# V2AI/EFG

Hardware: AMD Instinct MI355X
Metric: scenes/sec ConQueR 1-frame Waymo train step (higher is better)
Workload: dtype f32; 1 GPU; ConQueR res18 p3, 1-sweep Waymo-shaped scenes, 180000 pts/scene, 0.1 m voxels, 2 scenes/GPU, 900 queries, fwd+bwd+AdamW+OneCycle, graph of `value`: FPN levels / heads the reference evaluates and never reads are skipped (same losses and gradients; the line's `full_graph` object times the full reference graph); global_batch=2, parallelism=dp1

## Files before the change

efg_amd/_lib.py:

```python
import ctypes
import os

import torch

_LIB_PATH = os.path.join(os.path.dirname(os.path.abspath(__file__)), "lib", "libefg_hip.so")
_lib = None

c_void_p, c_int, c_int64, c_size_t, c_float = (ctypes.c_void_p, ctypes.c_int, ctypes.c_int64, ctypes.c_size_t,
                                               ctypes.c_float)

_SIGS = {
    "efg_last_error": (ctypes.c_char_p, []),
    "efg_version": (ctypes.c_char_p, []),
    "efg_capture_stream_create": (ctypes.c_int, [ctypes.POINTER(ctypes.c_void_p)]),
    "efg_capture_stream_destroy": (ctypes.c_int, [ctypes.c_void_p]),
    "efg_dynamic_voxelize_f32": (c_int, [c_void_p, c_int64, c_int, c_void_p, c_void_p, c_void_p, c_void_p]),
    "efg_hard_voxelize_workspace_bytes": (c_size_t, [c_int64, c_int, c_int, c_int, c_int, c_void_p, c_void_p]),
    "efg_hard_voxelize_f32": (c_int, [c_void_p, c_void_p, c_int, c_int, c_void_p, c_void_p, c_int, c_int, c_void_p,
                                      c_void_p, c_int, c_void_p, c_void_p, c_void_p, c_void_p, c_size_t, c_void_p]),
    "efg_hard_voxelize_debug_timeline": (c_size_t, [c_void_p]),
    "efg_scatter_workspace_bytes": (c_size_t, [c_int64, c_int, c_void_p]),
    "efg_scatter_index": (c_int, [c_void_p, c_int64, c_int, c_void_p, c_void_p, c_void_p, c_void_p, c_size_t,
                                  c_void_p]),
    "efg_scatter_reduce_workspace_bytes": (c_size_t, [c_int64, c_int]),
    "efg_scatter_reduce_f32": (c_int, [c_void_p, c_void_p, c_void_p, c_int64, c_int, c_int, c_int, c_int64, c_void_p,
                                       c_void_p, c_void_p, c_void_p, c_size_t, c_void_p]),
    "efg_scatter_backward_f32": (c_int, [c_void_p, c_void_p, c_void_p, c_void_p, c_void_p, c_void_p, c_int64, c_int64,
                                         c_int, c_int, c_void_p, c_size_t, c_void_p]),
    "efg_spconv_index_bytes": (c_size_t, [c_int, c_void_p]),
    "efg_spconv_index_workspace_bytes": (c_size_t, [c_int, c_void_p]),
    "efg_spconv_index_from_indices": (c_int, [c_void_p, c_int64, c_int, c_void_p, c_void_p, c_void_p, c_void_p,
                                              c_size_t, c_void_p]),
    "efg_spconv_index_downsample": (c_int, [c_void_p, c_int64, c_int, c_void_p, c_void_p, c_void_p, c_void_p,
                                            c_void_p, c_void_p, c_void_p, c_void_p, c_size_t, c_void_p]),
    "efg_spconv_index_rank": (c_int, [c_void_p, c_int, c_void_p, c_void_p, c_void_p, c_size_t, c_void_p]),
    "efg_spconv_index_emit": (c_int, [c_void_p, c_int, c_void_p, c_void_p, c_void_p]),
    "efg_spconv_build_nbr": (c_int, [c_void_p, c_void_p, c_int, c_void_p, c_void_p, c_int64, c_void_p, c_void_p,
                                     c_void_p, c_void_p, c_void_p]),
    "efg_spconv_build_rnbr": (c_int, [c_void_p, c_int64, c_int, c_int64, c_void_p, c_void_p]),
    "efg_spconv_packed_weight_bytes": (c_size_t, [c_int, c_int, c_int, c_int]),
    "efg_spconv_pack_weight_f32": (c_int, [c_void_p, c_int, c_int, c_int, c_int, c_void_p, c_void_p]),
    "efg_spconv_pack_weights_multi": (c_int, [c_void_p, c_int, c_void_p]),
    "efg_spconv_forward_f32": (c_int, [c_void_p, c_int64, c_int, c_void_p, c_void_p, c_int, c_int, c_void_p, c_int64,
                                       c_void_p, c_void_p]),
    "efg_spconv_dgrad_f32": (c_int, [c_void_p, c_int64, c_int, c_void_p, c_int, c_int, c_void_p, c_int64, c_void_p,
                                     c_void_p, c_void_p]),
    "efg_spconv_tile_plan_bytes": (c_size_t, [c_int64, c_int]),
    "efg_spconv_tile_plan": (c_int, [c_void_p, c_int64, c_int, c_void_p, c_size_t, c_void_p]),
    "efg_spconv_forward_tiled_f32": (c_int, [c_void_p, c_int64, c_int, c_void_p, c_void_p, c_int, c_int, c_void_p,
                                             c_int64, c_int, c_void_p, c_void_p]),
    "efg_spconv_tiled_pair_f32": (c_int, [c_void_p, c_void_p, c_int64, c_int, c_void_p, c_void_p, c_int, c_int, c_void_p,
                                          c_int64, c_int, c_void_p, c_void_p, c_void_p]),
    "efg_spconv_small_ok": (c_int, [c_int, c_int, c_int, c_void_p, c_void_p]),
    "efg_spconv_tile_bf16x3_ok": (c_int, [c_int, c_int, c_int, c_int64, c_int64]),
    "efg_spconv_streamk_fallbacks": (c_int, [c_void_p, c_int]),
    "efg_ticket_ring_errors": (c_int, [c_void_p, c_int]),
    "efg_spconv_parity_order": (c_int, [c_void_p, c_int64, c_void_p, c_void_p, c_size_t, c_void_p]),
    "efg_spconv_wgrad_workspace_bytes": (c_size_t, [c_int64, c_int, c_int, c_int]),
    "efg_spconv_wgrad_f32": (c_int, [c_void_p, c_int64, c_int, c_void_p, c_int64, c_int, c_int, c_void_p, c_void_p,
                                     c_void_p, c_size_t, c_void_p]),
    "efg_spconv_wgrad_tiled_ok": (c_int, [c_int, c_int, c_int]),
    "efg_spconv_wgrad_tiled_workspace_bytes": (c_size_t, [c_int64, c_int, c_int, c_int]),
    "efg_spconv_wgrad_sched_bytes": (c_size_t, [c_int64, c_int, c_int, c_int]),
    "efg_spconv_wgrad_sched": (c_int, [c_void_p, c_int64, c_int, c_int, c_int, c_void_p, c_size_t, c_void_p]),
    "efg_spconv_wgrad_tiled_f32": (c_int, [c_void_p, c_int64, c_int, c_void_p, c_int64, c_int, c_int, c_void_p,
                                           c_void_p, c_void_p, c_void_p, c_size_t, c_void_p]),
    "efg_spconv_wgrad_tiled_pair_f32": (c_int, [c_void_p, c_int64, c_int, c_void_p, c_void_p, c_int64, c_int, c_int, c_void_p,
                                                c_void_p, c_void_p, c_void_p, c_void_p, c_size_t, c_void_p]),
    "efg_sparse_to_dense_f32": (c_int, [c_void_p, c_int, c_void_p, c_void_p, c_int, c_void_p, c_void_p, c_void_p]),
    "efg_dense_to_sparse_f32": (c_int, [c_void_p, c_int, c_void_p, c_int64, c_int, c_void_p, c_void_p, c_void_p]),
    "efg_sparse_to_bev_f32": (c_int, [c_void_p, c_int, c_void_p, c_void_p, c_int, c_void_p, c_void_p, c_void_p]),
    "efg_bev_to_sparse_f32": (c_int, [c_void_p, c_int, c_void_p, c_int64, c_int, c_void_p, c_void_p, c_void_p]),
    "efg_msda_forward_f32": (c_int, [c_void_p, c_void_p, c_void_p, c_void_p, c_void_p, c_int, c_int, c_int, c_int,
                                     c_int, c_int, c_int, c_void_p, c_void_p]),
    "efg_msda_backward_f32": (c_int, [c_void_p, c_void_p, c_void_p, c_void_p, c_void_p, c_void_p, c_int, c_int, c_int,
                                      c_int, c_int, c_int, c_int, c_void_p, c_void_p, c_void_p, c_void_p]),
    "efg_box_attn_fused_forward_f32": (c_int, [c_void_p] * 7 + [c_int] * 8 + [c_void_p, c_void_p]),
    "efg_box_attn_fused_forward_strided_f32": (c_int, [c_void_p] * 5 + [c_int, c_void_p, c_int, c_void_p] + [c_int] * 8 + [c_void_p, c_void_p]),
    "efg_box_attn_fused_backward_strided_f32": (c_int, [c_void_p] * 5 + [c_int, c_void_p, c_int, c_void_p, c_void_p] + [c_int] * 8 + [c_void_p] * 4 + [c_size_t, c_void_p]),
    "efg_box_attn_fused_backward_workspace_bytes": (c_size_t, [c_int] * 6),
    "efg_box_attn_fused_backward_f32": (c_int, [c_void_p] * 8 + [c_int] * 8 + [c_void_p] * 4 + [c_size_t, c_void_p]),
    "efg_boxes_bev_f32": (c_int, [c_void_p, c_int, c_void_p, c_int, c_int, c_void_p, c_void_p]),
    "efg_nms_workspace_bytes": (c_size_t, [c_int]),
    "efg_topk_unsorted_f32": (c_int, [c_void_p, c_int64, c_int, c_int, c_void_p, c_void_p, c_void_p]),
    "efg_box_refine_forward_f32": (c_int, [c_void_p, c_void_p, c_int64, c_float, c_void_p, c_void_p]),
    "efg_box_refine_backward_f32": (c_int, [c_void_p, c_void_p, c_void_p, c_int64, c_float, c_void_p, c_void_p, c_void_p]),
    "efg_add_layernorm_forward_f32": (c_int, [c_void_p] * 4 + [c_float, c_int64, c_int] + [c_void_p] * 5),
    "efg_add_layernorm_backward_workspace_bytes": (c_size_t, [c_int64, c_int]),
    "efg_add_layernorm_backward_f32": (c_int, [c_void_p] * 5 + [c_int64, c_int] + [c_void_p] * 4 + [c_size_t, c_void_p]),
    "efg_points_transform_filter_workspace_bytes": (c_size_t, [c_int64]),
    "efg_points_transform_filter_f32": (c_int, [c_void_p, c_int64, c_int, c_void_p, c_int, c_void_p, c_void_p, c_void_p,
                                                c_void_p, c_size_t, c_void_p]),
    "efg_points_gather_f32": (c_int, [c_void_p, c_void_p, c_int64, c_int, c_void_p, c_void_p]),
    "efg_match_cost_f32": (c_int, [c_void_p] * 4 + [c_int] * 5 + [c_float] * 6 + [c_void_p, c_void_p]),
    "efg_focal_loss_forward_f32": (c_int, [c_void_p, c_void_p, c_int, c_int64, c_int, c_float, c_float, c_void_p, c_void_p,
                                           c_void_p]),
    "efg_focal_loss_backward_f32": (c_int, [c_void_p, c_void_p, c_int, c_int64, c_int, c_float, c_float, c_void_p,
                                            c_void_p, c_void_p, c_void_p]),
    "efg_box_loss_forward_f32": (c_int, [c_void_p] * 6 + [c_int64] + [c_int] * 4 + [c_void_p] * 3),
    "efg_box_loss_backward_f32": (c_int, [c_void_p] * 6 + [c_int64] + [c_int] * 4 + [c_void_p] * 4),
    "efg_bn_workspace_bytes": (c_size_t, [c_int]),
    "efg_bn_forward_f32": (c_int, [c_void_p] * 7 + [c_float, c_float, c_int64, c_int, c_int] + [c_void_p] * 4 +
                           [c_size_t, c_void_p]),
    "efg_bn_backward_f32": (c_int, [c_void_p] * 6 + [c_int64, c_int, c_int] + [c_void_p] * 5 + [c_size_t, c_void_p]),
    "efg_lsap_f32": (c_int, [c_void_p, c_int, c_int, c_int, c_void_p, c_void_p, c_void_p, c_void_p]),
    "efg_nms_f32": (c_int, [c_void_p, c_int, c_float, c_int, c_void_p, c_void_p, c_void_p, c_size_t, c_void_p]),
    "efg_spconv_tile_shape": (c_int, [c_int, c_int, c_int, c_int64, c_int64, c_void_p, c_void_p, c_void_p]),
    "efg_cylinder_select_f32": (c_int, [c_void_p, c_int64, c_int, c_int, c_float, c_void_p, c_void_p, c_int64, c_void_p,
                                        c_void_p, c_void_p, c_int, c_void_p, c_void_p]),
    "efg_attention_fwd_f32": (c_int, [c_void_p, c_int64, c_int64, c_void_p, c_void_p, c_int64, c_int64, c_int64, c_int, c_int,
                                      c_int, c_float, c_void_p, c_void_p, c_void_p]),
    "efg_attention_bwd_f32": (c_int, [c_void_p, c_int64, c_int64, c_void_p, c_void_p, c_int64, c_int64, c_void_p, c_void_p,
                                      c_void_p, c_int64, c_int, c_int, c_int, c_float, c_void_p, c_void_p, c_void_p,
                                      c_void_p]),
    "efg_attention_long_fwd_f32": (c_int, [c_void_p, c_int64, c_int64] * 3 + [c_void_p, c_int, c_int64, c_int, c_int, c_float,
                                                                             c_void_p, c_void_p, c_void_p]),
    "efg_attention_long_bwd_f32": (c_int, [c_void_p, c_int64, c_int64] * 3 + [c_void_p, c_int, c_void_p, c_void_p, c_void_p,
                                                                             c_int64, c_int, c_int, c_float, c_void_p, c_void_p,
                                                                             c_void_p, c_void_p, c_void_p]),
    "efg_relu_bwd_colsum_f32": (c_int, [c_void_p, c_void_p, c_int64, c_int, c_void_p, c_void_p, c_void_p, c_size_t, c_void_p]),
    "efg_nms_segmented_f32": (c_int, [c_void_p, c_void_p, c_int, c_float, c_int, c_void_p, c_void_p, c_void_p, c_size_t,
                                      c_void_p]),
    "efg_gn_workspace_bytes": (c_size_t, [c_int, c_int]),
    "efg_gn_forward_f32": (c_int, [c_void_p] * 3 + [c_float, c_int, c_int64, c_int, c_int] + [c_void_p] * 4 +
                           [c_size_t, c_void_p]),
    "efg_gn_backward_f32": (c_int, [c_void_p] * 5 + [c_int, c_int64, c_int, c_int] + [c_void_p] * 4 +
                            [c_size_t, c_void_p]),
    "efg_gemm_bf16x3_pack_bytes": (c_size_t, [c_int, c_int]),
    "efg_gemm_bf16x3_pack_f32": (c_int, [c_void_p, c_int64, c_int64, c_int, c_int, c_void_p, c_void_p]),
    "efg_gemm_bf16x3_pack_linear_f32": (c_int, [c_void_p, c_int, c_int, c_void_p, c_void_p, c_void_p]),
    "efg_gemm_bf16x3_f32": (c_int, [c_void_p, c_int64, c_int, c_int64, c_void_p, c_int, c_void_p, c_int, c_void_p, c_int64,
                                    c_void_p]),
    "efg_gemm_bf16x3_wgrad_workspace_bytes": (c_size_t, [c_int64, c_int, c_int]),
    "efg_gemm_bf16x3_wgrad_f32": (c_int, [c_void_p, c_int64, c_void_p, c_int64, c_int64, c_int, c_int, c_void_p, c_void_p,
                                          c_size_t, c_void_p]),
    "efg_gemm_bf16x6_pack_bytes": (c_size_t, [c_int, c_int]),
    "efg_gemm_bf16x6_pack_f32": (c_int, [c_void_p, c_int64, c_int64, c_int, c_int, c_void_p, c_void_p]),
    "efg_gemm_bf16x6_pack_linear_f32": (c_int, [c_void_p, c_int, c_int, c_void_p, c_void_p, c_void_p]),
    "efg_gemm_bf16x6_f32": (c_int, [c_void_p, c_int64, c_int, c_int64, c_void_p, c_int, c_void_p, c_int, c_void_p, c_int64,
                                    c_void_p]),
    "efg_gemm_bf16x6_wgrad_workspace_bytes": (c_size_t, [c_int64, c_int, c_int]),
    "efg_gemm_bf16x6_wgrad_f32": (c_int, [c_void_p, c_int64, c_void_p, c_int64, c_int64, c_int, c_int, c_void_p, c_void_p,
                                          c_size_t, c_void_p]),
    "efg_colsum_workspace_bytes": (c_size_t, [c_int64, c_int]),
    "efg_colsum_f32": (c_int, [c_void_p, c_int64, c_int, c_int64, c_void_p, c_void_p, c_size_t, c_void_p]),
}

EXPORTED_SYMBOLS = tuple(_SIGS)


def lib_path():
    return _LIB_PATH


def _warn_if_stale():
    csrc = os.path.join(os.path.dirname(os.path.abspath(__file__)), "csrc")
    try:
        built = os.path.getmtime(_LIB_PATH)
        newer = [f for f in os.listdir(csrc) if os.path.getmtime(os.path.join(csrc, f)) > built + 1.0]
    except OSError:
        return
    if newer:
        import warnings

        warnings.warn("efg_amd: %s is OLDER than %s -- rebuild with `python -m efg_amd.build`"
                      % (os.path.basename(_LIB_PATH), ", ".join(sorted(newer)[:4])), RuntimeWarning, stacklevel=3)


def lib():
    global _lib
    if _lib is None:
        if not os.path.exists(_LIB_PATH):
            raise RuntimeError(
                "efg_amd: %s is missing. Build it with `python -m efg_amd.build` (hipcc, gfx950). "
                "There is no CPU fallback on the product path." % _LIB_PATH)
        _warn_if_stale()
        ab = os.environ.get("EFG_HIP_LIB_AB")
        path = os.path.join(os.path.dirname(_LIB_PATH), os.path.basename(ab)) if ab else _LIB_PATH
        if ab and not os.path.exists(path):
            raise RuntimeError("efg_amd: EFG_HIP_LIB_AB=%s not found in %s" % (ab, os.path.dirname(_LIB_PATH)))
        _lib = ctypes.CDLL(path)
        for name, (res, args) in _SIGS.items():
            fn = getattr(_lib, name)
            fn.restype = res
            fn.argtypes = args
    return _lib


def check(rc):
    if rc != 0:
        raise RuntimeError("efg_hip: " + lib().efg_last_error().decode())


def ptr(t):
    if t is None:
        return None
    assert t.is_contiguous(), "efg_hip ops need contiguous tensors"
    return t.data_ptr()


def stream():
    raw = getattr(torch._C, "_cuda_getCurrentRawStream", None)
    if raw is not None:
        return raw(torch.cuda.current_device())
    return torch.cuda.current_stream().cuda_stream


def require_gpu(*tensors):
    for t in tensors:
        if t is not None and not t.is_cuda:
            raise RuntimeError(
                "efg_amd ops run on MI355X only (got a %s tensor); there is no CPU fallback" % t.device.type)


def host_f32(vals, n):
    vals = [float(v) for v in vals]
    assert len(vals) == n
    return (ctypes.c_float * n)(*vals)


def host_i32(vals, n=None):
    vals = [int(v) for v in vals]
    assert n is None or len(vals) == n
    return (ctypes.c_int * len(vals))(*vals)


def host_i64(vals):
    vals = [int(v) for v in vals]
    return (ctypes.c_int64 * len(vals))(*vals)
```

efg_amd/build.py:

```python
import os
import subprocess
import sys

_PKG = os.path.dirname(os.path.abspath(__file__))
_ROOT = os.path.dirname(_PKG)
CSRC = os.path.join(_PKG, "csrc")
LIB_DIR = os.path.join(_PKG, "lib")
LIB_PATH = os.path.join(LIB_DIR, "libefg_hip.so")

SOURCES = ["lib.cpp", "voxelize.hip", "voxelize_bins.hip", "voxelize_hash.hip", "scatter.hip", "spconv_index.hip", "spconv_conv.hip", "spconv_tiles.hip", "spconv_wgt.hip", "msda.hip", "box_fused.hip", "iou3d_nms.hip", "matcher.hip", "layernorm.hip", "augment.hip", "det_loss.hip", "batchnorm.hip", "colsum.hip", "crop.hip", "attention.hip", "gemm_bf16x3.hip", "gemm_bf16x6.hip", "topk.hip"]
FLAGS = ["--offload-arch=gfx950", "-O3", "-std=c++17", "-fPIC", "-munsafe-fp-atomics", "-ffp-contract=off",
         "-Wall", "-Wno-unused-function", "-I" + os.path.join(_ROOT, "include"), "-I" + CSRC]


def _stale(target, deps):
    if not os.path.exists(target):
        return True
    t = os.path.getmtime(target)
    return any(os.path.getmtime(d) > t for d in deps)


def build(force=False, verbose=False):
    os.makedirs(LIB_DIR, exist_ok=True)
    hipcc = os.environ.get("HIPCC", "/opt/rocm/bin/hipcc")
    headers = [os.path.join(CSRC, h) for h in os.listdir(CSRC) if h.endswith(".h")]
    headers.append(os.path.join(_ROOT, "include", "efg_hip.h"))
    objs = []
    procs = []
    for src in SOURCES:
        path = os.path.join(CSRC, src)
        if not os.path.exists(path):
            continue
        obj = os.path.join(LIB_DIR, os.path.splitext(src)[0] + ".o")
        objs.append(obj)
        if force or _stale(obj, [path] + headers):
            cmd = [hipcc] + FLAGS + ["-x", "hip", "-c", path, "-o", obj]
            if verbose:
                print(" ".join(cmd))
            procs.append((src, subprocess.Popen(cmd, stdout=subprocess.PIPE, stderr=subprocess.STDOUT)))
    for src, p in procs:
        out, _ = p.communicate()
        if p.returncode != 0:
            raise RuntimeError("hipcc failed on %s:\n%s" % (src, out.decode()))
        if verbose and out:
            print(out.decode())
    if force or procs or _stale(LIB_PATH, objs):
        cmd = [hipcc, "--offload-arch=gfx950", "-shared", "-fPIC", "-o", LIB_PATH] + objs
        subprocess.check_call(cmd)
    return LIB_PATH


if __name__ == "__main__":
    print(build(force="--force" in sys.argv, verbose=True))
```

efg_amd/detection3d/optimizer.py:

```python
import torch


class CachedFusedAdamW(torch.optim.AdamW):

    def __init__(self, params, **kw):
        kw["fused"] = True
        super().__init__(params, **kw)
        self._plan = None

    def _plain(self, group):
        return not (group["amsgrad"] or group["maximize"] or group["capturable"] or group["differentiable"]
                    or torch.is_tensor(group["lr"]))

    def _build_plan(self):
        plan = []
        for group in self.param_groups:
            params, grads, exp_avgs, exp_avg_sqs, max_sqs, steps = [], [], [], [], [], []
            self._init_group(group, params, grads, exp_avgs, exp_avg_sqs, max_sqs, steps)
            assert len({(p.device, p.dtype) for p in params}) <= 1, "one device / dtype per group"
            plan.append((params, exp_avgs, exp_avg_sqs, steps))
        return plan

    @torch.no_grad()
    def step(self, closure=None):
        if closure is not None or not all(self._plain(g) for g in self.param_groups):
            return super().step(closure)
        if self._plan is None:
            self._plan = self._build_plan()
        todo = []
        for group, (params, exp_avgs, exp_avg_sqs, steps) in zip(self.param_groups, self._plan):
            grads = [p.grad for p in params]
            if any(g is None for g in grads) or len(params) != sum(p.grad is not None for p in group["params"]):
                self._plan = None
                return super().step()
            todo.append((group, params, grads, exp_avgs, exp_avg_sqs, steps))
        found_inf = getattr(self, "found_inf", None)
        for group, params, grads, exp_avgs, exp_avg_sqs, steps in todo:
            if not params:
                continue
            beta1, beta2 = group["betas"]
            torch._foreach_add_(steps, 1)
            torch._fused_adamw_(params, grads, exp_avgs, exp_avg_sqs, [], steps, amsgrad=False, lr=group["lr"],
                                beta1=beta1, beta2=beta2, weight_decay=group["weight_decay"], eps=group["eps"],
                                maximize=False, grad_scale=None, found_inf=found_inf)
            if found_inf is not None:
                torch._foreach_sub_(steps, [found_inf.reshape(()).to(steps[0].dtype)] * len(steps))
        return None


def build_adamw_multi(cfg, model):
    oc = dict(cfg.solver.optimizer)
    oc.pop("type", None)
    lr = oc["lr"]
    lr_backbone = oc.pop("lr_backbone", lr)
    named = [(n, p) for n, p in model.named_parameters() if p.requires_grad]
    backbone = [p for p in model.backbone.parameters() if p.requires_grad]
    rest = [p for n, p in named if "backbone" not in n and "linear_box" not in n]
    deform = [p for n, p in named if "linear_box" in n and "backbone" not in n]
    groups = [{"params": backbone, "lr": lr_backbone}, {"params": rest},
              {"params": deform, "lr": lr * cfg.solver.deform_lr_multi}]
    oc["betas"] = tuple(oc["betas"])
    if all(p.is_cuda for g in groups for p in g["params"]):
        return CachedFusedAdamW(groups, **oc)
    return torch.optim.AdamW(groups, **oc)
```

include/efg_hip.h:

```cpp
#ifndef EFG_HIP_H
#define EFG_HIP_H
#include <stddef.h>
#include <stdint.h>

#ifdef __cplusplus
extern "C" {
#endif

#define EFG_OK 0
#define EFG_E_INVALID (-1)
#define EFG_E_WORKSPACE (-2)
#define EFG_E_HIP (-3)

const char* efg_last_error(void);
const char* efg_version(void);

int efg_capture_stream_create(void** stream_out);
int efg_capture_stream_destroy(void* stream);


int efg_dynamic_voxelize_f32(const float* points, int64_t n, int f, const float* voxel_size_host,
                             const float* coors_range_host, int32_t* coors, void* stream);

size_t efg_hard_voxelize_workspace_bytes(int64_t n_total, int batch, int f, int max_points, int max_voxels,
                                         const float* voxel_size_host, const float* coors_range_host);

int efg_hard_voxelize_f32(const float* points, const int64_t* point_offsets_host, int batch, int f,
                          const float* voxel_size_host, const float* coors_range_host, int max_points,
                          int max_voxels, float* voxels, int32_t* coors, int coors_cols, int32_t* npv,
                          int32_t* voxel_num, float* mean, void* ws, size_t ws_bytes, void* stream);

size_t efg_hard_voxelize_debug_timeline(void* device_buf_u64);

size_t efg_scatter_workspace_bytes(int64_t n, int ndim, const int32_t* dims_host);
int efg_scatter_index(const int32_t* coors, int64_t n, int ndim, const int32_t* dims_host,
                      int32_t* point2voxel, int32_t* m_dev, void* ws, size_t ws_bytes, void* stream);
size_t efg_scatter_reduce_workspace_bytes(int64_t m, int c);
int efg_scatter_reduce_f32(const float* feats, const int32_t* coors, const int32_t* point2voxel, int64_t n,
                           int c, int ndim, int reduce, int64_t m, float* voxel_feats, int32_t* voxel_coors,
                           int32_t* count, void* ws, size_t ws_bytes, void* stream);
int efg_scatter_backward_f32(float* grad_feats, const float* grad_voxel_feats, const float* feats,
                             const float* voxel_feats, const int32_t* point2voxel, const int32_t* count,
                             int64_t n, int64_t m, int c, int reduce, void* ws, size_t ws_bytes, void* stream);

size_t efg_spconv_index_bytes(int batch, const int* shape_host);
size_t efg_spconv_index_workspace_bytes(int batch, const int* shape_host);

int efg_spconv_index_from_indices(const int32_t* indices, int64_t m, int batch, const int* shape_host,
                                  void* index, int32_t* perm, void* ws, size_t ws_bytes, void* stream);

int efg_spconv_index_downsample(const int32_t* in_indices, int64_t m_in, int batch, const int* in_shape_host,
                                const int* ksize_host, const int* stride_host, const int* pad_host,
                                void* out_index, int* out_shape_host, int32_t* m_out_dev, void* ws,
                                size_t ws_bytes, void* stream);
int efg_spconv_index_rank(void* index, int batch, const int* shape_host, int32_t* m_dev, void* ws, size_t ws_bytes,
                          void* stream);
int efg_spconv_index_emit(const void* index, int batch, const int* shape_host, int32_t* out_indices,
                          void* stream);

int efg_spconv_build_nbr(const void* in_index, const int32_t* in_perm, int batch, const int* in_shape_host,
                         const int32_t* out_indices, int64_t m_out, const int* ksize_host,
                         const int* stride_host, const int* pad_host, int32_t* nbr, void* stream);
int efg_spconv_build_rnbr(const int32_t* nbr, int64_t m_out, int kvol, int64_t m_in, int32_t* rnbr,
                          void* stream);

size_t efg_spconv_packed_weight_bytes(int cout, int kvol, int cin, int for_dgrad);
int efg_spconv_pack_weight_f32(const float* weight, int cout, int kvol, int cin, int for_dgrad, float* packed,
                               void* stream);
int efg_spconv_pack_weights_multi(const void* items_dev, int n, void* stream);

int efg_spconv_forward_f32(const float* in_feat, int64_t m_in, int cin, const float* packed_weight,
                           const float* bias, int cout, int kvol, const int32_t* nbr, int64_t m_out,
                           float* out_feat, void* stream);
int efg_spconv_dgrad_f32(const float* grad_out, int64_t m_out, int cout, const float* packed_weight, int cin,
                         int kvol, const int32_t* rnbr, int64_t m_in, const int32_t* row_order, float* grad_in,
                         void* stream);
size_t efg_spconv_tile_plan_bytes(int64_t m, int kvol);
int efg_spconv_tile_plan(const int32_t* nbr, int64_t m, int kvol, void* plan, size_t plan_bytes, void* stream);
int efg_spconv_tile_shape(int cin, int cout, int kvol, int64_t m_in, int64_t m_out, int* nt, int* r, int* ks);
int efg_spconv_forward_tiled_f32(const float* in_feat, int64_t m_in, int cin, const float* packed_weight,
                                 const float* bias, int cout, int kvol, const void* plan, int64_t m_out,
                                 int flip_offsets, float* out_feat, void* stream);
int efg_spconv_tiled_pair_f32(const float* in_a, const float* in_b, int64_t m_in, int cin, const float* packed_a,
                              const float* packed_b, int cout, int kvol, const void* plan, int64_t m_out, int flip_offsets,
                              float* out_a, float* out_b, void* stream);
int efg_spconv_streamk_fallbacks(int64_t* count_out, int reset);
int efg_spconv_small_ok(int cin, int cout, int kvol, int* c16, int* nt);
int efg_spconv_tile_bf16x3_ok(int cin, int cout, int kvol, int64_t m_in, int64_t m_out);

int efg_spconv_parity_order(const int32_t* indices, int64_t m, int32_t* order, void* ws, size_t ws_bytes,
                            void* stream);
size_t efg_spconv_wgrad_workspace_bytes(int64_t m_out, int cin, int cout, int kvol);
int efg_spconv_wgrad_f32(const float* in_feat, int64_t m_in, int cin, const float* grad_out, int64_t m_out,
                         int cout, int kvol, const int32_t* nbr, float* grad_w, void* ws, size_t ws_bytes,
                         void* stream);
int efg_spconv_wgrad_tiled_ok(int cin, int cout, int kvol);
size_t efg_spconv_wgrad_sched_bytes(int64_t m_out, int cin, int cout, int kvol);
int efg_spconv_wgrad_sched(const void* plan, int64_t m_out, int cin, int cout, int kvol, void* sched, size_t sched_bytes,
                           void* stream);
size_t efg_spconv_wgrad_tiled_workspace_bytes(int64_t m_out, int cin, int cout, int kvol);
int efg_spconv_wgrad_tiled_f32(const float* in_feat, int64_t m_in, int cin, const float* grad_out, int64_t m_out,
                               int cout, int kvol, const void* plan, const void* sched, float* grad_w, void* ws,
                               size_t ws_bytes, void* stream);
int efg_spconv_wgrad_tiled_pair_f32(const float* in_feat, int64_t m_in, int cin, const float* grad_out_a,
                                    const float* grad_out_b, int64_t m_out, int cout, int kvol, const void* plan,
                                    const void* sched, float* grad_w_a, float* grad_w_b, void* ws, size_t ws_bytes,
                                    void* stream);

int efg_sparse_to_dense_f32(const float* feat, int c, const void* index, const int32_t* perm, int batch,
                            const int* shape_host, float* dense, void* stream);
int efg_dense_to_sparse_f32(const float* grad_dense, int c, const int32_t* indices, int64_t m, int batch,
                            const int* shape_host, float* grad_feat, void* stream);

int efg_sparse_to_bev_f32(const float* feat, int c, const void* index, const int32_t* perm, int batch,
                          const int* shape_host, float* out, void* stream);
int efg_bev_to_sparse_f32(const float* grad_out, int c, const int32_t* indices, int64_t m, int batch,
                          const int* shape_host, float* grad_feat, void* stream);

int efg_msda_forward_f32(const float* value, const int64_t* shapes, const int64_t* level_start,
                         const float* loc, const float* attn, int b, int s, int h, int d, int l, int lq, int p,
                         float* out, void* stream);
int efg_msda_backward_f32(const float* value, const int64_t* shapes, const int64_t* level_start,
                          const float* loc, const float* attn, const float* grad_out, int b, int s, int h,
                          int d, int l, int lq, int p, float* grad_value, float* grad_loc, float* grad_attn,
                          void* stream);

int efg_box_attn_fused_forward_f32(const float* value, const int64_t* shapes, const int64_t* level_start,
                                   const float* ref_windows, const float* offsets, const float* logits,
                                   const float* kernel_indices, int b, int s, int h, int d, int l, int lq, int p,
                                   int v, float* out, void* stream);
size_t efg_box_attn_fused_backward_workspace_bytes(int b, int s, int h, int l, int lq, int p);
int efg_box_attn_fused_backward_f32(const float* value, const int64_t* shapes, const int64_t* level_start,
                                    const float* ref_windows, const float* offsets, const float* logits,
                                    const float* kernel_indices, const float* grad_out, int b, int s, int h, int d,
                                    int l, int lq, int p, int v, float* grad_value, float* grad_offsets,
                                    float* grad_logits, void* ws, size_t ws_bytes, void* stream);

int efg_ticket_ring_errors(int64_t* count_out, int reset);

int efg_box_attn_fused_forward_strided_f32(const float* value, const int64_t* shapes, const int64_t* level_start,
                                           const float* ref_windows, const float* offsets, int off_row_stride,
                                           const float* logits, int logit_row_stride, const float* kernel_indices, int b,
                                           int s, int h, int d, int l, int lq, int p, int v, float* out, void* stream);
int efg_box_attn_fused_backward_strided_f32(const float* value, const int64_t* shapes, const int64_t* level_start,
                                            const float* ref_windows, const float* offsets, int off_row_stride,
                                            const float* logits, int logit_row_stride, const float* kernel_indices,
                                            const float* grad_out, int b, int s, int h, int d, int l, int lq, int p, int v,
                                            float* grad_value, float* grad_offsets, float* grad_logits, void* ws,
                                            size_t ws_bytes, void* stream);

int efg_boxes_bev_f32(const float* boxes_a, int na, const float* boxes_b, int nb, int mode, float* out,
                      void* stream);
size_t efg_nms_workspace_bytes(int n);
int efg_nms_f32(const float* boxes_sorted, int n, float thresh, int rotated, int64_t* keep, int* num_keep,
                void* ws, size_t ws_bytes, void* stream);
int efg_nms_segmented_f32(const float* boxes_sorted, const int32_t* segment, int n, float thresh, int rotated,
                          int64_t* keep, int* num_keep, void* ws, size_t ws_bytes, void* stream);

int efg_cylinder_select_f32(const float* points, int64_t n_points, int f, int time_col, float max_time,
                            const int64_t* point_range, const float* centre_radius, int64_t n_cyl, const int64_t* starts,
                            int32_t* counts, int32_t* index, int n_chunks, int32_t* chunk_counts, void* stream);

int efg_attention_fwd_f32(const float* q, int64_t q_batch_stride, int64_t q_row_stride, const float* k, const float* v,
                          int64_t kv_batch_stride, int64_t kv_row_stride, int64_t batch, int seq_q, int seq_k, int heads,
                          float scale, float* out, float* lse, void* stream);
int efg_attention_bwd_f32(const float* q, int64_t q_batch_stride, int64_t q_row_stride, const float* k, const float* v,
                          int64_t kv_batch_stride, int64_t kv_row_stride, const float* out, const float* lse,
                          const float* dout, int64_t batch, int seq_q, int seq_k, int heads, float scale, float* dq, float* dk,
                          float* dv, void* stream);

int efg_attention_long_fwd_f32(const float* q, int64_t q_batch_stride, int64_t q_row_stride, const float* k,
                               int64_t k_batch_stride, int64_t k_row_stride, const float* v, int64_t v_batch_stride,
                               int64_t v_row_stride, const uint32_t* mask_bits, int mask_words, int64_t batch, int s, int heads,
                               float scale, float* out, float* lse, void* stream);
int efg_attention_long_bwd_f32(const float* q, int64_t q_batch_stride, int64_t q_row_stride, const float* k,
                               int64_t k_batch_stride, int64_t k_row_stride, const float* v, int64_t v_batch_stride,
                               int64_t v_row_stride, const uint32_t* mask_bits, int mask_words, const float* out,
                               const float* lse, const float* dout, int64_t batch, int s, int heads, float scale, float* dq,
                               float* dk, float* dv, float* delta_ws , void* stream);

int efg_lsap_f32(const float* cost, int n_problems, int nq, int g_stride, const int32_t* ng,
                 int64_t* query_of_gt, int32_t* status, void* stream);

int efg_add_layernorm_forward_f32(const float* x, const float* residual, const float* gamma, const float* beta,
                                  float eps, int64_t rows, int c, float* z_out, float* y, float* mean, float* rstd,
                                  void* stream);
size_t efg_add_layernorm_backward_workspace_bytes(int64_t rows, int c);
int efg_add_layernorm_backward_f32(const float* dy, const float* z, const float* mean, const float* rstd,
                                   const float* gamma, int64_t rows, int c, float* dz, float* dgamma, float* dbeta,
                                   void* ws, size_t ws_bytes, void* stream);

enum { EFG_PT_NEG_Y = 0,
       EFG_PT_NEG_X = 1,
       EFG_PT_ROT_Z = 2,
       EFG_PT_SCALE = 3,
       EFG_PT_TRANSLATE = 4  };
typedef struct { int kind; float a, b, c; } efg_point_op;
size_t efg_points_transform_filter_workspace_bytes(int64_t n);
int efg_points_transform_filter_f32(const float* points, int64_t n, int f, const efg_point_op* ops_host, int n_ops,
                                    const float* range_host, float* out, int32_t* count, void* ws, size_t ws_bytes,
                                    void* stream);
int efg_points_gather_f32(const float* points, const int64_t* index, int64_t m, int f, float* out, void* stream);

int efg_match_cost_f32(const float* logits, const float* boxes, const int64_t* tgt_labels, const float* tgt_boxes,
                       int p, int b, int q, int c, int g, float w_class, float w_bbox, float w_giou, float w_rad,
                       float alpha, float gamma, float* cost, void* stream);
int efg_focal_loss_forward_f32(const float* logits, const int32_t* target_class, int layers, int64_t n, int c,
                               float alpha, float gamma, const float* denom, float* out, void* stream);
int efg_focal_loss_backward_f32(const float* logits, const int32_t* target_class, int layers, int64_t n, int c,
                                float alpha, float gamma, const float* denom, const float* grad_out,
                                float* grad_logits, void* stream);
int efg_box_loss_forward_f32(const float* boxes, const float* tgt_boxes, const int64_t* l_idx, const int64_t* b_idx,
                             const int64_t* q_idx, const int64_t* g_idx, int64_t n, int layers, int b, int q, int g,
                             const float* denom, float* out, void* stream);
int efg_box_loss_backward_f32(const float* boxes, const float* tgt_boxes, const int64_t* l_idx, const int64_t* b_idx,
                              const int64_t* q_idx, const int64_t* g_idx, int64_t n, int layers, int b, int q, int g,
                              const float* denom, const float* grad_out, float* grad_boxes, void* stream);

int efg_topk_unsorted_f32(const float* x, int64_t rows, int n, int k, float* values, int64_t* indices, void* stream);

int efg_box_refine_forward_f32(const float* delta, const float* anchor, int64_t n, float eps, float* out, void* stream);
int efg_box_refine_backward_f32(const float* grad, const float* out, const float* anchor, int64_t n, float eps,
                                float* grad_delta, float* grad_anchor, void* stream);

size_t efg_bn_workspace_bytes(int c);
int efg_bn_forward_f32(const float* x, const float* residual, const float* weight, const float* bias,
                       float* running_mean, float* running_var, int64_t* num_batches_tracked, float momentum, float eps,
                       int64_t m, int c, int relu, float* y, float* mean, float* invstd, void* ws, size_t ws_bytes,
                       void* stream);
int efg_bn_backward_f32(const float* dy, const float* x, const float* y, const float* weight, const float* mean,
                        const float* invstd, int64_t m, int c, int relu, float* dx, float* dresidual, float* dweight,
                        float* dbias, void* ws, size_t ws_bytes, void* stream);

size_t efg_gn_workspace_bytes(int batch, int c);
int efg_gn_forward_f32(const float* x, const float* weight, const float* bias, float eps, int batch, int64_t rows,
                       int c, int groups, float* y, float* mean, float* rstd, void* ws, size_t ws_bytes, void* stream);
int efg_gn_backward_f32(const float* dy, const float* x, const float* weight, const float* mean, const float* rstd,
                        int batch, int64_t rows, int c, int groups, float* dx, float* dweight, float* dbias, void* ws,
                        size_t ws_bytes, void* stream);

size_t efg_colsum_workspace_bytes(int64_t rows, int cols);
int efg_colsum_f32(const float* x, int64_t rows, int cols, int64_t row_stride, float* out, void* ws, size_t ws_bytes,
                   void* stream);
int efg_relu_bwd_colsum_f32(const float* g, const float* y, int64_t rows, int cols, float* g_out, float* out, void* ws,
                            size_t ws_bytes, void* stream);

size_t efg_gemm_bf16x3_pack_bytes(int k, int n);
int efg_gemm_bf16x3_pack_f32(const float* w, int64_t stride_k, int64_t stride_n, int k, int n, void* packed,
                             void* stream);
int efg_gemm_bf16x3_pack_linear_f32(const float* w, int n_out, int n_in, void* packed_fwd, void* packed_dgrad, void* stream);
int efg_gemm_bf16x3_f32(const float* a, int64_t m, int k, int64_t lda, const void* packed_b, int n, const float* bias,
                        int relu, float* c, int64_t ldc, void* stream);
size_t efg_gemm_bf16x3_wgrad_workspace_bytes(int64_t m, int n, int k);
int efg_gemm_bf16x3_wgrad_f32(const float* g, int64_t ldg, const float* x, int64_t ldx, int64_t m, int n, int k, float* dw,
                              void* ws, size_t ws_bytes, void* stream);

size_t efg_gemm_bf16x6_pack_bytes(int k, int n);
int efg_gemm_bf16x6_pack_f32(const float* w, int64_t stride_k, int64_t stride_n, int k, int n, void* packed,
                             void* stream);
int efg_gemm_bf16x6_pack_linear_f32(const float* w, int n_out, int n_in, void* packed_fwd, void* packed_dgrad, void* stream);
int efg_gemm_bf16x6_f32(const float* a, int64_t m, int k, int64_t lda, const void* packed_b, int n, const float* bias,
                        int relu, float* c, int64_t ldc, void* stream);
size_t efg_gemm_bf16x6_wgrad_workspace_bytes(int64_t m, int n, int k);
int efg_gemm_bf16x6_wgrad_f32(const float* g, int64_t ldg, const float* x, int64_t ldx, int64_t m, int n, int k, float* dw,
                              void* ws, size_t ws_bytes, void* stream);

#ifdef __cplusplus
}
#endif
#endif
```

Before: 64.49 scenes/s.

## Replace per-group fused AdamW with a single custom HIP launch over all params

Adds a HIP AdamW kernel driven by a pinned host table of pointers, per-group scalars and a chunk-to-tensor map, so all parameters are updated in one kernel launch. It replaces the per-group torch foreach step-increment and fused AdamW launches. Step counters are updated in-kernel using atomic tickets so only the last chunk of each tensor writes the step. The cost is a small host-to-device table copy each step, a ring of events to avoid overwriting pinned buffers still in flight, and double-precision coefficient math meant to match PyTorch numerics.

```diff
diff --git a/efg_amd/_lib.py b/efg_amd/_lib.py
--- a/efg_amd/_lib.py
+++ b/efg_amd/_lib.py
@@ -144,6 +144,9 @@
                                           c_size_t, c_void_p]),
     "efg_colsum_workspace_bytes": (c_size_t, [c_int64, c_int]),
     "efg_colsum_f32": (c_int, [c_void_p, c_int64, c_int, c_int64, c_void_p, c_void_p, c_size_t, c_void_p]),
+    "efg_adamw_chunk_elems": (c_int, []),
+    "efg_adamw_table_bytes": (c_size_t, [c_int, c_int, c_int64]),
+    "efg_adamw_step_f32": (c_int, [c_void_p, c_void_p, c_size_t, c_int, c_int, c_int64, c_void_p, c_void_p]),
 }
 
 EXPORTED_SYMBOLS = tuple(_SIGS)
diff --git a/efg_amd/build.py b/efg_amd/build.py
--- a/efg_amd/build.py
+++ b/efg_amd/build.py
@@ -8,7 +8,7 @@
 LIB_DIR = os.path.join(_PKG, "lib")
 LIB_PATH = os.path.join(LIB_DIR, "libefg_hip.so")
 
-SOURCES = ["lib.cpp", "voxelize.hip", "voxelize_bins.hip", "voxelize_hash.hip", "scatter.hip", "spconv_index.hip", "spconv_conv.hip", "spconv_tiles.hip", "spconv_wgt.hip", "msda.hip", "box_fused.hip", "iou3d_nms.hip", "matcher.hip", "layernorm.hip", "augment.hip", "det_loss.hip", "batchnorm.hip", "colsum.hip", "crop.hip", "attention.hip", "gemm_bf16x3.hip", "gemm_bf16x6.hip", "topk.hip"]
+SOURCES = ["lib.cpp", "voxelize.hip", "voxelize_bins.hip", "voxelize_hash.hip", "scatter.hip", "spconv_index.hip", "spconv_conv.hip", "spconv_tiles.hip", "spconv_wgt.hip", "msda.hip", "box_fused.hip", "iou3d_nms.hip", "matcher.hip", "layernorm.hip", "augment.hip", "det_loss.hip", "batchnorm.hip", "colsum.hip", "crop.hip", "attention.hip", "gemm_bf16x3.hip", "gemm_bf16x6.hip", "topk.hip", "adamw.hip"]
 FLAGS = ["--offload-arch=gfx950", "-O3", "-std=c++17", "-fPIC", "-munsafe-fp-atomics", "-ffp-contract=off",
          "-Wall", "-Wno-unused-function", "-I" + os.path.join(_ROOT, "include"), "-I" + CSRC]
 
diff --git a/efg_amd/csrc/adamw.hip b/efg_amd/csrc/adamw.hip
--- /dev/null
+++ b/efg_amd/csrc/adamw.hip
@@ -0,0 +1,125 @@
+#include "common.h"
+
+namespace efg {
+namespace {
+
+constexpr int kChunk = 16384;
+constexpr int kTensorWords = 8;
+constexpr int kGroupWords = 8;
+
+struct Coef {
+  double beta1, beta2, omb1, omb2, lrwd, eps;
+  float step_size, bc2_sqrt;
+  bool decay;
+};
+
+__device__ __forceinline__ void adamw_one(const Coef& k, float& p, float g, float& m, float& v) {
+  const double pd = (double)p, gd = (double)g;
+  if (k.decay) p = (float)__fma_rn(-k.lrwd, pd, pd);
+  m = (float)__fma_rn(k.beta1, (double)m, __dmul_rn(k.omb1, gd));
+  v = (float)__fma_rn(k.beta2, (double)v, __dmul_rn(__dmul_rn(k.omb2, gd), gd));
+  const float denom = (float)__dadd_rn((double)__fdiv_rn(sqrtf(v), k.bc2_sqrt), k.eps);
+  p = __fsub_rn(p, __fdiv_rn(__fmul_rn(k.step_size, m), denom));
+}
+
+__global__ void __launch_bounds__(256)
+adamw_kernel(const long long* __restrict__ table, int T, int G, const float* __restrict__ found_inf,
+             unsigned* __restrict__ tickets) {
+  const float fi = found_inf ? *found_inf : 0.f;
+  if (fi == 1.f) return;
+  const long long* rows = table + (long long)kGroupWords * G;
+  const long long where = rows[(long long)kTensorWords * T + blockIdx.x];
+  const int t = (int)(where & 0xffffffffll), chunk = (int)(where >> 32);
+  const long long numel = rows[5ll * T + t];
+  float* __restrict__ param = reinterpret_cast<float*>(rows[t]);
+  const float* __restrict__ grad = reinterpret_cast<const float*>(rows[1ll * T + t]);
+  float* __restrict__ exp_avg = reinterpret_cast<float*>(rows[2ll * T + t]);
+  float* __restrict__ exp_sq = reinterpret_cast<float*>(rows[3ll * T + t]);
+  float* step_ptr = reinterpret_cast<float*>(rows[4ll * T + t]);
+  const double* grp = reinterpret_cast<const double*>(table) + (long long)kGroupWords * rows[6ll * T + t];
+  const int chunks = (int)rows[7ll * T + t];
+
+  const float step = __fadd_rn(*step_ptr, 1.0f);
+  const double lr = grp[0], wd = grp[3];
+  Coef k;
+  k.beta1 = grp[1];
+  k.beta2 = grp[2];
+  k.omb1 = __dsub_rn(1.0, k.beta1);
+  k.omb2 = __dsub_rn(1.0, k.beta2);
+  k.lrwd = __dmul_rn(lr, wd);
+  k.eps = grp[4];
+  k.decay = wd != 0.0;
+  const float bc1 = (float)__dsub_rn(1.0, pow(k.beta1, (double)step));
+  k.bc2_sqrt = (float)__dsqrt_rn(__dsub_rn(1.0, pow(k.beta2, (double)step)));
+  k.step_size = (float)__ddiv_rn(lr, (double)bc1);
+
+  const long long base = (long long)chunk * kChunk;
+  const int n = (int)min((long long)kChunk, numel - base);
+  param += base;
+  grad += base;
+  exp_avg += base;
+  exp_sq += base;
+  const int n4 = n >> 2;
+  const bool grad_vec = (reinterpret_cast<uintptr_t>(grad) & 15) == 0;
+  for (int i = threadIdx.x; i < n4; i += 256) {
+    float4 p = reinterpret_cast<const float4*>(param)[i];
+    const float4 g = grad_vec ? reinterpret_cast<const float4*>(grad)[i]
+                              : make_float4(grad[4 * i], grad[4 * i + 1], grad[4 * i + 2], grad[4 * i + 3]);
+    float4 m = reinterpret_cast<const float4*>(exp_avg)[i];
+    float4 v = reinterpret_cast<const float4*>(exp_sq)[i];
+    adamw_one(k, p.x, g.x, m.x, v.x);
+    adamw_one(k, p.y, g.y, m.y, v.y);
+    adamw_one(k, p.z, g.z, m.z, v.z);
+    adamw_one(k, p.w, g.w, m.w, v.w);
+    reinterpret_cast<float4*>(param)[i] = p;
+    reinterpret_cast<float4*>(exp_avg)[i] = m;
+    reinterpret_cast<float4*>(exp_sq)[i] = v;
+  }
+  for (int i = (n4 << 2) + threadIdx.x; i < n; i += 256) {
+    float p = param[i], m = exp_avg[i], v = exp_sq[i];
+    adamw_one(k, p, grad[i], m, v);
+    param[i] = p;
+    exp_avg[i] = m;
+    exp_sq[i] = v;
+  }
+
+  __syncthreads();
+  if (threadIdx.x == 0) {
+    bool last = true;
+    if (chunks > 1) {
+      const unsigned prev = __hip_atomic_fetch_add(tickets + t, 1u, __ATOMIC_ACQ_REL, __HIP_MEMORY_SCOPE_AGENT);
+      last = prev == (unsigned)chunks - 1;
+      if (last) __hip_atomic_store(tickets + t, 0u, __ATOMIC_RELAXED, __HIP_MEMORY_SCOPE_AGENT);
+    }
+    if (last) *step_ptr = found_inf ? __fsub_rn(step, fi) : step;
+  }
+}
+
+}
+}
+
+using namespace efg;
+
+extern "C" int efg_adamw_chunk_elems(void) { return kChunk; }
+
+extern "C" size_t efg_adamw_table_bytes(int n_tensors, int n_groups, int64_t n_blocks) {
+  if (n_tensors < 1 || n_groups < 1 || n_blocks < 1) return 0;
+  return sizeof(long long) * ((size_t)kGroupWords * n_groups + (size_t)kTensorWords * n_tensors + (size_t)n_blocks);
+}
+
+extern "C" int efg_adamw_step_f32(const void* host_table, void* dev_table, size_t table_bytes, int n_tensors, int n_groups,
+                                  int64_t n_blocks, const float* found_inf, void* stream) {
+  EFG_CHECK_ARG(n_tensors >= 1 && n_groups >= 1 && n_blocks >= 1 && n_blocks <= 0x7fffffffll,
+                "adamw: need at least one tensor, group and block (got %d, %d, %lld)", n_tensors, n_groups, (long long)n_blocks);
+  EFG_CHECK_ARG(host_table && dev_table, "adamw: null table");
+  EFG_CHECK_ARG(table_bytes == efg_adamw_table_bytes(n_tensors, n_groups, n_blocks), "adamw: table is %zu bytes, expected %zu",
+                table_bytes, efg_adamw_table_bytes(n_tensors, n_groups, n_blocks));
+  hipStream_t st = (hipStream_t)stream;
+  unsigned* tickets = ticket_slots(n_tensors, st);
+  EFG_CHECK_ARG(tickets, "adamw: no ticket slots (more than 2048 tensors, or a stream that is being captured)");
+  EFG_HIP_TRY(hipMemcpyAsync(dev_table, host_table, table_bytes, hipMemcpyHostToDevice, st));
+  hipLaunchKernelGGL(adamw_kernel, dim3((unsigned)n_blocks), dim3(256), 0, st, static_cast<const long long*>(dev_table),
+                     n_tensors, n_groups, found_inf, tickets);
+  EFG_LAUNCH_CHECK();
+  return EFG_OK;
+}
diff --git a/efg_amd/detection3d/optimizer.py b/efg_amd/detection3d/optimizer.py
--- a/efg_amd/detection3d/optimizer.py
+++ b/efg_amd/detection3d/optimizer.py
@@ -1,4 +1,86 @@
+import os
+
+import numpy as np
 import torch
+
+from .. import _lib
+
+
+def _dense(t):
+    n = 1
+    for size, stride in sorted(((s, st) for s, st in zip(t.shape, t.stride()) if s != 1), key=lambda x: x[1]):
+        if stride != n:
+            return False
+        n *= size
+    return True
+
+
+class _OneLaunchPlan:
+    RING = 4
+
+    def __init__(self, groups, plan):
+        lib = _lib.lib()
+        chunk = lib.efg_adamw_chunk_elems()
+        self.params, self.exp_avgs, self.exp_avg_sqs, self.steps, self.group_of = [], [], [], [], []
+        self.stock = []
+        for gi, (params, exp_avgs, exp_avg_sqs, steps) in enumerate(plan):
+            rest = []
+            for i, (p, m, v, s) in enumerate(zip(params, exp_avgs, exp_avg_sqs, steps)):
+                ok = (p.dtype == m.dtype == v.dtype == s.dtype == torch.float32 and s.numel() == 1 and s.device == p.device
+                      and p.numel() > 0 and _dense(p) and m.stride() == p.stride() == v.stride()
+                      and m.shape == p.shape == v.shape
+                      and not (p.data_ptr() | m.data_ptr() | v.data_ptr()) & 15 and not s.data_ptr() & 3)
+                if ok:
+                    self.params.append(p), self.exp_avgs.append(m), self.exp_avg_sqs.append(v), self.steps.append(s)
+                    self.group_of.append(gi)
+                else:
+                    rest.append(i)
+            self.stock.append(rest)
+        self.n, self.n_groups = len(self.params), len(groups)
+        if not self.n or self.n > 2048 or len({p.device for p in self.params}) != 1:
+            self.n = 0
+            return
+        self.device = self.params[0].device
+        self.param_ptrs = [p.data_ptr() for p in self.params]
+        self.numel = np.array([p.numel() for p in self.params], np.int64)
+        chunks = (self.numel + chunk - 1) // chunk
+        self.n_blocks = int(chunks.sum())
+        words = 8 * self.n_groups + 8 * self.n + self.n_blocks
+        assert lib.efg_adamw_table_bytes(self.n, self.n_groups, self.n_blocks) == 8 * words
+        tensor_of = np.repeat(np.arange(self.n, dtype=np.int64), chunks)
+        chunk_of = np.arange(self.n_blocks, dtype=np.int64) - np.repeat(np.cumsum(chunks) - chunks, chunks)
+        self.host = [torch.empty(words, dtype=torch.int64).pin_memory() for _ in range(self.RING)]
+        self.events = [None] * self.RING
+        self.turn = 0
+        for h in self.host:
+            t = h.numpy()
+            t[:8 * self.n_groups] = 0
+            rows = t[8 * self.n_groups:8 * self.n_groups + 8 * self.n].reshape(8, self.n)
+            for r, tensors in enumerate((self.params, None, self.exp_avgs, self.exp_avg_sqs, self.steps)):
+                if tensors is not None:
+                    rows[r] = self.param_ptrs if r == 0 else [x.data_ptr() for x in tensors]
+            rows[5], rows[6], rows[7] = self.numel, self.group_of, chunks
+            t[8 * self.n_groups + 8 * self.n:] = tensor_of | (chunk_of << 32)
+        self.dev = torch.empty(words, dtype=torch.int64, device=self.device)
+
+    def launch(self, groups, grad_ptrs, found_inf):
+        k = self.turn
+        self.turn = (k + 1) % self.RING
+        if self.events[k] is not None:
+            self.events[k].synchronize()
+        t = self.host[k].numpy()
+        scal = t[:8 * self.n_groups].view(np.float64).reshape(self.n_groups, 8)
+        for gi, g in enumerate(groups):
+            scal[gi, :5] = (g["lr"], g["betas"][0], g["betas"][1], g["weight_decay"], g["eps"])
+        rows = t[8 * self.n_groups:8 * self.n_groups + 8 * self.n].reshape(8, self.n)
+        rows[1] = grad_ptrs
+        with torch.cuda.device(self.device):
+            _lib.check(_lib.lib().efg_adamw_step_f32(self.host[k].data_ptr(), self.dev.data_ptr(), 8 * t.size, self.n,
+                                                     self.n_groups, self.n_blocks,
+                                                     None if found_inf is None else found_inf.data_ptr(), _lib.stream()))
+            if self.events[k] is None:
+                self.events[k] = torch.cuda.Event()
+            self.events[k].record()
 
 
 class CachedFusedAdamW(torch.optim.AdamW):
@@ -7,6 +89,7 @@
         kw["fused"] = True
         super().__init__(params, **kw)
         self._plan = None
+        self._one = None
 
     def _plain(self, group):
         return not (group["amsgrad"] or group["maximize"] or group["capturable"] or group["differentiable"]
@@ -27,6 +110,7 @@
             return super().step(closure)
         if self._plan is None:
             self._plan = self._build_plan()
+            self._one = None
         todo = []
         for group, (params, exp_avgs, exp_avg_sqs, steps) in zip(self.param_groups, self._plan):
             grads = [p.grad for p in params]
@@ -35,6 +119,8 @@
                 return super().step()
             todo.append((group, params, grads, exp_avgs, exp_avg_sqs, steps))
         found_inf = getattr(self, "found_inf", None)
+        if os.environ.get("EFG_ADAMW_ONE_LAUNCH", "1") != "0" and not torch.cuda.is_current_stream_capturing():
+            todo = self._step_one_launch(todo, found_inf)
         for group, params, grads, exp_avgs, exp_avg_sqs, steps in todo:
             if not params:
                 continue
@@ -46,6 +132,34 @@
             if found_inf is not None:
                 torch._foreach_sub_(steps, [found_inf.reshape(()).to(steps[0].dtype)] * len(steps))
         return None
+
+    def _step_one_launch(self, todo, found_inf):
+        if self._one is None:
+            self._one = _OneLaunchPlan(self.param_groups, self._plan)
+        one = self._one
+        if not one.n or (found_inf is not None and not (found_inf.dtype == torch.float32 and found_inf.numel() == 1
+                                                        and found_inf.device == one.device)):
+            return todo
+        if [p.data_ptr() for p in one.params] != one.param_ptrs:
+            self._plan = None
+            return todo
+        grads = [p.grad for p in one.params]
+        ptrs = [g.data_ptr() for g in grads]
+        if any(g.stride() != p.stride() or g.dtype != torch.float32 or a & 3 or g.shape != p.shape or g.device != p.device
+               for p, g, a in zip(one.params, grads, ptrs)):
+            return todo
+        one.launch(self.param_groups, ptrs, found_inf)
+        if not any(one.stock):
+            return []
+        return [(group, *([lst[i] for i in stock] for lst in lists)) for (group, *lists), stock in zip(todo, one.stock)]
+
+    def load_state_dict(self, state_dict):
+        super().load_state_dict(state_dict)
+        self._plan = None
+
+    def add_param_group(self, param_group):
+        super().add_param_group(param_group)
+        self._plan = None
 
 
 def build_adamw_multi(cfg, model):
diff --git a/include/efg_hip.h b/include/efg_hip.h
--- a/include/efg_hip.h
+++ b/include/efg_hip.h
@@ -265,6 +265,11 @@
 int efg_gemm_bf16x6_wgrad_f32(const float* g, int64_t ldg, const float* x, int64_t ldx, int64_t m, int n, int k, float* dw,
                               void* ws, size_t ws_bytes, void* stream);
 
+int efg_adamw_chunk_elems(void);
+size_t efg_adamw_table_bytes(int n_tensors, int n_groups, int64_t n_blocks);
+int efg_adamw_step_f32(const void* host_table, void* dev_table, size_t table_bytes, int n_tensors, int n_groups,
+                       int64_t n_blocks, const float* found_inf, void* stream);
+
 #ifdef __cplusplus
 }
 #endif
```

New measurement: 64.98 scenes/s (median of 5 runs). About the same (+0.8%).
